# michaelriedl/2048-ppo-agent

Hardware: AMD Instinct MI355X
Metric: env-steps/sec at N parallel boards (full PPO loop: rollout with policy in the loop + GAE + update) (higher is better)
Workload: dtype u8 boards / bf16 policy; 1 GPU; 65536 parallel boards per GPU, Transformer policy bf16 (3.96 M params), full PPO iteration (BASELINE.json configs[2]; configs[3] when n_gpus=8); boards_per_gpu=65536, global_boards=65536, train_batch=2048, update_epochs=5, max_samples_per_epoch=300000, max_samples_per_epoch_is=global (each rank draws its 1/N share), as the reference's single subset, max_samples_per_epoch_per_rank=300000, rollout_mode=episodes (reference lock-step semantics), rng_mode=partitionable, parallelism=env-shard x1 + 1 grad all-reduce/minibatch

## Files before the change

### 2048-ppo-agent_amd/csrc/g2048_policy.hip

```cpp
#include <hip/hip_runtime.h>
#include <stdint.h>

#include "../../include/g2048.h"
#include "g2048_host.h"
#include "g2048_mfma.h"

namespace {

using g2048_mfma::bf16x4;
using g2048_mfma::bf16x8;
using g2048_mfma::f32x16;
using g2048_mfma::f32x4;
using g2048_mfma::mfma;
using g2048_mfma::rowof;
using g2048_mfma::sched_fence;
using g2048_mfma::static_for;
using namespace g2048_host;

typedef short s16x2 __attribute__((ext_vector_type(2)));

constexpr int D = 256, NH = 8, HD = 32, FF = 1024, SEQ = 17, NBOARD = 7, NTOK = 128, THREADS = 256;
constexpr int W_LAYER = 3 * D * D + D * D + FF * D + D * FF;
constexpr int P_LAYER = D + D + 3 * D + D + D + D + FF + D;
constexpr int WO_QKV = 0, WO_O = 3 * D * D, WO_1 = WO_O + D * D, WO_2 = WO_1 + FF * D;
constexpr int PO_LN1G = 0, PO_LN1B = D, PO_BQKV = 2 * D, PO_BO = 5 * D, PO_LN2G = 6 * D, PO_LN2B = 7 * D,
              PO_B1 = 8 * D, PO_B2 = 8 * D + FF;
constexpr int FFC = 64;
constexpr int TILE = 32 * D * 2;
constexpr float SM_SCALE_LOG2E = 0.17677669529663687f * 1.4426950408889634f;

template <int CPR> __device__ __forceinline__ int swz(int r);
template <> __device__ __forceinline__ int swz<32>(int r) { return r & 15; }
template <> __device__ __forceinline__ int swz<16>(int r) { return r & 15; }
template <> __device__ __forceinline__ int swz<8>(int r) { return (r >> 1) & 7; }
template <> __device__ __forceinline__ int swz<4>(int r) { return (r >> 2) & 3; }

struct LaneOff {
    int a256[8];
    int a64[4];
    int a32[2];
    unsigned s256[2], s64, s32;
};
__device__ __forceinline__ void lane_offsets(LaneOff &o, int r, int h, int w, int lane) {
    for (int k = 0; k < 8; ++k) o.a256[k] = r * 512 + (((2 * k + h) ^ swz<32>(r)) * 16);
    for (int k = 0; k < 4; ++k) o.a64[k] = r * 128 + (((2 * k + h) ^ swz<8>(r)) * 16);
    for (int k = 0; k < 2; ++k) o.a32[k] = r * 64 + (((2 * k + h) ^ swz<4>(r)) * 16);
    for (int par = 0; par < 2; ++par) {
        const int x = 2 * w + (lane >> 5), row15 = (8 * par + x) & 15;
        o.s256[par] = (unsigned)(x * D * 2 + (((lane & 31) ^ row15) * 16));
    }
    {
        const int x = 8 * w + (lane >> 3);
        o.s64 = (unsigned)(x * FF * 2 + (((lane & 7) ^ swz<8>(x)) * 16));
    }
    {
        const int x = 16 * w + (lane >> 2);
        o.s32 = (unsigned)(x * D * 2 + (((lane & 3) ^ swz<4>(x)) * 16));
    }
}

template <int CPR>
__device__ __forceinline__ bf16x8 load_w(const char *tile, const LaneOff &o, int mt, int ks) {
    if (CPR == 32) return *reinterpret_cast<const bf16x8 *>(tile + o.a256[ks & 7] + (ks >> 3) * 256 + mt * 32 * 512);
    if (CPR == 8) return *reinterpret_cast<const bf16x8 *>(tile + o.a64[ks] + mt * 32 * 128);
    return *reinterpret_cast<const bf16x8 *>(tile + o.a32[ks] + mt * 32 * 64);
}
__device__ __forceinline__ bf16x8 load_p(const char *row, int ks, int h) {
    return *reinterpret_cast<const bf16x8 *>(row + 2 * (16 * ks + 8 * h));
}

__device__ __forceinline__ void frag_from_acc(const f32x16 &x, bf16x8 out[2]) {
    for (int s = 0; s < 2; ++s)
        for (int j = 0; j < 8; ++j) out[s][j] = (__bf16)x[8 * s + j];
}
__device__ __forceinline__ void relu_frag_from_acc(const f32x16 &x, bf16x8 out[2]) {
    frag_from_acc(x, out);
    for (int s = 0; s < 2; ++s) {
        s16x2 *p = reinterpret_cast<s16x2 *>(&out[s]);
        const s16x2 zero = {0, 0};
        for (int q = 0; q < 4; ++q) p[q] = __builtin_elementwise_max(p[q], zero);
    }
}

__device__ __forceinline__ f32x16 bias_tile(const float *b32, int h) {
    f32x16 a;
    for (int g = 0; g < 4; ++g) {
        const f32x4 v = *reinterpret_cast<const f32x4 *>(b32 + 8 * g + 4 * h);
        for (int q = 0; q < 4; ++q) a[4 * g + q] = v[q];
    }
    return a;
}

template <int CPR, int NK, bool SWAP = false>
__device__ __forceinline__ f32x16 gemm_tile(const char *tile, const LaneOff &o, int mt, const bf16x8 *b, f32x16 acc) {
    bf16x8 a[NK];
    for (int ks = 0; ks < NK; ++ks) a[ks] = load_w<CPR>(tile, o, mt, ks);
    for (int ks = 0; ks < NK; ++ks) acc = SWAP ? mfma(b[ks], a[ks], acc) : mfma(a[ks], b[ks], acc);
    return acc;
}
template <int NM, int EXTRA = 0, int NV = 0, int VALU_PER = 0, int TRANS_PER = 0, int DEPTH = 8>
__device__ __forceinline__ void pipe_mfma() {
    __builtin_amdgcn_sched_group_barrier(0x100, DEPTH + EXTRA, 0);
#pragma unroll
    for (int i = 0; i < NM; ++i) {
        __builtin_amdgcn_sched_group_barrier(0x008, 1, 0);
        if (i < NM - DEPTH) __builtin_amdgcn_sched_group_barrier(0x100, 1, 0);
        if (i < NV && VALU_PER) __builtin_amdgcn_sched_group_barrier(0x002, VALU_PER, 0);
        if (i < NV && TRANS_PER) __builtin_amdgcn_sched_group_barrier(0x400, TRANS_PER, 0);
    }
}

#ifdef G2048_STAMPS
constexpr int N_STAMPS = 24;
__device__ unsigned long long g_stamps[N_STAMPS];
struct StampSite {
    __device__ __forceinline__ static bool on(int lane, int w) { return lane == 0 && w == 0 && blockIdx.x % 64 == 0; }
    __device__ __forceinline__ static unsigned long long *table(int) { return g_stamps; }
};
#define STAMP(k) stamps.mark(k)
#else
#define STAMP(k)
#endif

typedef __amdgpu_buffer_rsrc_t rsrc_t;
template <int CPR>
__device__ __forceinline__ void dma_tile(char *dst, rsrc_t blob, unsigned src_byte, int ld, int rows, const LaneOff &o, int w) {
    const int n_inst = rows * CPR / (64 * 4);
    const int rows_per_inst = 4 * 64 / CPR;
    for (int t = 0; t < n_inst; ++t) {
        const unsigned lane_off = CPR == 32 ? o.s256[t & 1] : (CPR == 8 ? o.s64 : o.s32);
        __builtin_amdgcn_raw_ptr_buffer_load_lds(blob, (__attribute__((address_space(3))) void *)(dst + (t * 4 + w) * 1024), 16,
                                                 (int)lane_off, (int)(src_byte + (unsigned)(t * rows_per_inst * ld * 2)), 0, 0);
    }
}
template <int CPR>
__device__ __forceinline__ void dma_inst(char *dst, rsrc_t blob, unsigned src_byte, int ld, int t, const LaneOff &o, int w) {
    const int rows_per_inst = 4 * 64 / CPR;
    const unsigned lane_off = CPR == 32 ? o.s256[t & 1] : (CPR == 8 ? o.s64 : o.s32);
    __builtin_amdgcn_raw_ptr_buffer_load_lds(blob, (__attribute__((address_space(3))) void *)(dst + (t * 4 + w) * 1024), 16,
                                             (int)lane_off, (int)(src_byte + (unsigned)(t * rows_per_inst * ld * 2)), 0, 0);
}
template <int N> __device__ __forceinline__ void dma_wait() { asm volatile("s_waitcnt vmcnt(%0)" ::"n"(N) : "memory"); }
__device__ __forceinline__ void dma_wait_all() { dma_wait<0>(); }

__device__ __forceinline__ void stage_f32(float *dst, const float *src, int n, int tid) {
    for (int i = tid; i < n; i += THREADS) dst[i] = src[i];
}

__device__ __forceinline__ void park_in_agpr(bf16x8 &x) { asm volatile("" : "+a"(x)); }

__device__ __forceinline__ float xhalf_sum(float x) {
    const auto r = __builtin_amdgcn_permlane32_swap(__float_as_uint(x), __float_as_uint(x), false, false);
    return __uint_as_float(r[0]) + __uint_as_float(r[1]);
}
__device__ __forceinline__ float xhalf_max(float x) {
    const auto r = __builtin_amdgcn_permlane32_swap(__float_as_uint(x), __float_as_uint(x), false, false);
    return fmaxf(__uint_as_float(r[0]), __uint_as_float(r[1]));
}

__device__ __forceinline__ void layer_norm(const f32x16 r[8], bf16x8 out[16]) {
    typedef float f32x2 __attribute__((ext_vector_type(2)));
    f32x2 s2[4], q2[4];
    for (int k = 0; k < 4; ++k) s2[k] = q2[k] = f32x2{0.f, 0.f};
    for (int j = 0; j < 8; ++j)
        for (int i = 0; i < 16; i += 2) {
            const f32x2 v = {r[j][i], r[j][i + 1]};
            const int k = (i >> 1) & 3;
            s2[k] += v;
            q2[k] = __builtin_elementwise_fma(v, v, q2[k]);
        }
    const f32x2 st = (s2[0] + s2[1]) + (s2[2] + s2[3]), qt = (q2[0] + q2[1]) + (q2[2] + q2[3]);
    float s = st[0] + st[1], ss = qt[0] + qt[1];
    s = xhalf_sum(s);
    ss = xhalf_sum(ss);
    const float mean = s * (1.0f / D);
    const float var = fmaxf(__builtin_fmaf(-mean, mean, ss * (1.0f / D)), 0.0f);
    const float rstd = rsqrtf(var + 1e-5f), shift = -mean * rstd;
    for (int j = 0; j < 8; ++j)
        for (int i = 0; i < 16; ++i) out[2 * j + (i >> 3)][i & 7] = (__bf16)__builtin_fmaf(r[j][i], rstd, shift);
    for (int k = 0; k < 16; ++k) park_in_agpr(out[k]);
}

constexpr int MODE_FULL = 0, MODE_HEAD = 1, MODE_MEAN = 2;
constexpr int64_t KV_ELEMS = (int64_t)NH * SEQ * HD;

constexpr int L_WQKV = 0;
constexpr int L_WO = 6 * TILE;
constexpr int L_K = 7 * TILE;
constexpr int L_VT = 7 * TILE + TILE / 2;
constexpr int L_W1 = 0;
constexpr int L_W2 = 4 * TILE;
struct LdsMain {
    char w[8 * TILE];
    float bq[D], bo[D], b1[FF], b2[D];
};
static_assert(sizeof(LdsMain) <= 160 * 1024, "LDS budget");
constexpr int MEAN_LD = D + 4;
static_assert(NBOARD * 16 * MEAN_LD * 4 <= (int)sizeof(LdsMain::w), "mean-pool stage fits over the weight area");

template <int MODE>
__global__ void __launch_bounds__(THREADS, 1)
k_encoder_main(const uint8_t *__restrict__ boards, const float *__restrict__ table, const float *__restrict__ cls,
               const __bf16 *__restrict__ wblob, const float *__restrict__ pblob, int n_layers,
               float *__restrict__ features, int64_t B, __bf16 *__restrict__ ws_k, __bf16 *__restrict__ ws_v,
               float *__restrict__ ws_r) {
    extern __shared__ __attribute__((aligned(16))) char smem[];
    LdsMain &L = *reinterpret_cast<LdsMain *>(smem);
    const int tid = threadIdx.x, lane = tid & 63, r = lane & 31, h = lane >> 5;
    const int w = __builtin_amdgcn_readfirstlane(tid >> 6);
    const int64_t board0 = (int64_t)blockIdx.x * NBOARD;
    LaneOff lo;
    lane_offsets(lo, r, h, w, lane);

    const int tok = 32 * w + r;
    const int tb = tok / SEQ;
    const int tc = tok - tb * SEQ;
    const bool tok_valid = tb < NBOARD && board0 + tb < B;

    const int kb = w == 0 ? 0 : (w == 1 ? 16 : (w == 2 ? 48 : 64));
    int k_rd[2], vt_rd[4], k_wr[2], vt_wr[2];
    for (int ks = 0; ks < 2; ++ks) k_rd[ks] = L_K + kb * 64 + lo.a32[ks];
    for (int ks = 0; ks < 4; ++ks) vt_rd[ks] = L_VT + r * 256 + (((kb / 8 + 2 * ks + h) ^ swz<16>(r)) * 16);
    for (int s = 0; s < 2; ++s) {
        k_wr[s] = L_K + tok * 64 + (((2 * s + h) ^ swz<4>(tok)) * 16);
        vt_wr[s] = L_VT + r * 256 + (((4 * w + 2 * s + h) ^ swz<16>(r)) * 16);
    }
    bf16x8 kmask[2], qmask;
    {
        const int qb = tb;
        for (int j = 0; j < 8; ++j) qmask[j] = (__bf16)((qb == 8 * h + j) ? 16.0f : 0.0f);
        for (int tl = 0; tl < 2; ++tl) {
            const int kbd = (kb + 32 * tl + r) / SEQ;
            for (int j = 0; j < 8; ++j) kmask[tl][j] = (__bf16)((kbd == 8 * h + j) ? 16.0f : 0.0f);
        }
        park_in_agpr(qmask);
        park_in_agpr(kmask[0]);
        park_in_agpr(kmask[1]);
    }

    f32x16 R[8];
    {
        const float *src = cls;
        if (tok_valid && tc != 0) {
            int e = boards[(board0 + tb) * 16 + (tc - 1)];
            e = e > 30 ? 30 : e;
            src = table + ((size_t)(tc - 1) * 31 + e) * D;
        }
        const float keep = tok_valid ? 1.0f : 0.0f;
        for (int j = 0; j < 8; ++j)
            for (int g = 0; g < 4; ++g) {
                const f32x4 v = *reinterpret_cast<const f32x4 *>(src + 32 * j + 8 * g + 4 * h);
                for (int q = 0; q < 4; ++q) R[j][4 * g + q] = keep * v[q];
            }
    }

    const int full_layers = MODE == MODE_HEAD ? n_layers - 1 : n_layers;
    char *const lds = L.w;
    const rsrc_t blob = __builtin_amdgcn_make_buffer_rsrc(const_cast<__bf16 *>(wblob), 0, n_layers * (W_LAYER * 2), 0x00020000);
    auto wqkv = [&](int hd) -> char * { return lds + L_WQKV + (hd & 1) * 3 * TILE; };
    auto dma_qkv1 = [&](unsigned lw, int hd, int n) __attribute__((always_inline)) {
        dma_inst<32>(wqkv(hd) + (n / 4) * TILE, blob, lw + 2u * (unsigned)(WO_QKV + ((n / 4) * D + HD * hd) * D), D, n % 4, lo, w);
    };
    auto dma_wo1 = [&](unsigned lw, int hd, int n) __attribute__((always_inline)) {
        dma_inst<4>(lds + L_WO, blob, lw + 2u * (unsigned)(WO_O + HD * hd), D, n, lo, w);
    };
    auto dma_w11 = [&](unsigned lw, int c, int n) __attribute__((always_inline)) {
        dma_inst<32>(lds + L_W1 + (c & 1) * 2 * TILE, blob, lw + 2u * (unsigned)(WO_1 + FFC * c * D), D, n, lo, w);
    };
    auto dma_w21 = [&](unsigned lw, int c, int n) __attribute__((always_inline)) {
        dma_inst<8>(lds + L_W2 + (c & 1) * 2 * TILE, blob, lw + 2u * (unsigned)(WO_2 + FFC * c), FF, n, lo, w);
    };

#ifdef G2048_STAMPS
    g2048_mfma::Stamps<N_STAMPS, StampSite> stamps;
    stamps.start();
#endif
    for (int n = 0; n < 12; ++n) dma_qkv1(0u, 0, n);
    for (int n = 0; n < 12; ++n) dma_qkv1(0u, 1, n);

    constexpr int PD = 8;
    bf16x8 xn[16];
#pragma nounroll
    for (int layer = 0; layer < full_layers; ++layer) {
        const unsigned lw = (unsigned)layer * (unsigned)(W_LAYER * 2);
        const float *P = pblob + (size_t)layer * P_LAYER;

        float stg[7];
        stg[0] = P[PO_BQKV + tid];
        stg[1] = P[PO_BO + tid];
        stg[2] = P[PO_B2 + tid];
        for (int q = 0; q < 4; ++q) stg[3 + q] = P[PO_B1 + 256 * q + tid];
        layer_norm(R, xn);
        L.bq[tid] = stg[0];
        L.bo[tid] = stg[1];
        L.b2[tid] = stg[2];
        for (int q = 0; q < 4; ++q) L.b1[256 * q + tid] = stg[3 + q];
        dma_wait_all();
        __syncthreads();
        STAMP(0);

        f32x16 qa, ka, va;
        bf16x8 qf[2], kf[2], vf[2];
        auto project = [&](int hd, auto softmax_tag, auto fetch, f32x16 &s0, f32x16 &s1, bf16x8 *pf, float &sum) __attribute__((always_inline)) {
            constexpr bool SOFTMAX = decltype(softmax_tag)::value;
            const char *t = wqkv(hd);
            bf16x8 a[PD];
            qa = bias_tile(L.bq + HD * hd, h);
            for (int i = 0; i < 16; ++i) ka[i] = va[i] = 0.f;
            static_for<0, PD>([&](auto ic) __attribute__((always_inline)) {
                constexpr int i = decltype(ic)::value;
                a[i] = load_w<32>(t + (i / 16) * TILE, lo, 0, i % 16);
            });
            float m = 0.f, mc = 0.f;
            sched_fence();
            static_for<0, 48>([&](auto ic) __attribute__((always_inline)) {
                constexpr int i = decltype(ic)::value;
                constexpr int ks = i % 16;
                if constexpr (i < 16) qa = mfma(a[i % PD], xn[ks], qa);
                else if constexpr (i < 32) ka = mfma(a[i % PD], xn[ks], ka);
                else va = mfma(xn[ks], a[i % PD], va);
                if constexpr (i + PD < 48) a[i % PD] = load_w<32>(t + ((i + PD) / 16) * TILE, lo, 0, (i + PD) % 16);
                if constexpr (i % 3 == 0) fetch(std::integral_constant<int, i / 3>{});
                if constexpr (SOFTMAX) {
                    if constexpr (i < 8) {
                        const float x = fmaxf(fmaxf(s0[2 * i], s0[2 * i + 1]), fmaxf(s1[2 * i], s1[2 * i + 1]));
                        m = i == 0 ? x : fmaxf(m, x);
                    } else if constexpr (i == 8) {
                        m = xhalf_max(m);
                        mc = -m * SM_SCALE_LOG2E;
                        sum = 0.f;
                    } else if constexpr (i < 41) {
                        constexpr int e = i - 9;
                        if constexpr (e < 16) {
                            s0[e] = __builtin_amdgcn_exp2f(__builtin_fmaf(s0[e], SM_SCALE_LOG2E, mc));
                            sum += s0[e];
                        } else {
                            s1[e - 16] = __builtin_amdgcn_exp2f(__builtin_fmaf(s1[e - 16], SM_SCALE_LOG2E, mc));
                            sum += s1[e - 16];
                        }
                    } else if constexpr (i == 41) {
                        sum = xhalf_sum(sum);
                    } else if constexpr (i < 46) {
                        constexpr int k = i - 42;
                        for (int j = 0; j < 8; ++j) {
                            if constexpr (k < 2) pf[k][j] = (__bf16)s0[8 * (k & 1) + j];
                            else pf[k][j] = (__bf16)s1[8 * (k & 1) + j];
                        }
                    }
                }
                sched_fence();
            });
        };
        auto pack_qkv = [&](auto nc) __attribute__((always_inline)) {
            constexpr int n = decltype(nc)::value, which = n / 4, s = (n / 2) & 1, half = n & 1;
            for (int j = 0; j < 4; ++j) {
                if constexpr (which == 0) qf[s][4 * half + j] = (__bf16)qa[8 * s + 4 * half + j];
                else if constexpr (which == 1) kf[s][4 * half + j] = (__bf16)ka[8 * s + 4 * half + j];
                else vf[s][4 * half + j] = (__bf16)va[8 * s + 4 * half + j];
            }
        };
        auto store_kv = [&]() __attribute__((always_inline)) {
            for (int s = 0; s < 2; ++s) {
                *reinterpret_cast<bf16x8 *>(lds + k_wr[s]) = kf[s];
                *reinterpret_cast<bf16x8 *>(lds + vt_wr[s]) = vf[s];
            }
        };
        {
            f32x16 d0, d1;
            float dsum;
            project(0, std::false_type{}, [](auto) {}, d0, d1, nullptr, dsum);
            static_for<0, 12>(pack_qkv);
        }
        store_kv();
        __syncthreads();
        STAMP(1);

        auto head = [&](int hd, auto next_tag) __attribute__((always_inline)) {
            constexpr int NEXT = decltype(next_tag)::value;
            bf16x8 kr[4];
            for (int ks = 0; ks < 2; ++ks) {
                kr[2 * ks] = *reinterpret_cast<const bf16x8 *>(lds + k_rd[ks]);
                kr[2 * ks + 1] = *reinterpret_cast<const bf16x8 *>(lds + k_rd[ks] + 32 * 64);
            }
            sched_fence();
            auto fetch = [&](auto nc) __attribute__((always_inline)) {
                constexpr int n = decltype(nc)::value;
                if constexpr (n < 4) dma_wo1(lw, hd, n);
                else if constexpr (NEXT == 0) dma_qkv1(lw, hd + 2, n - 4);
                else if constexpr (NEXT == 1 && n < 12) dma_w11(lw, 0, n - 4);
            };
            if constexpr (NEXT == 2) static_for<0, 4>(fetch);
            sched_fence();
            STAMP(2);
            f32x16 s0 = {0}, s1 = {0};
            for (int ks = 0; ks < 2; ++ks) {
                s0 = mfma(kr[2 * ks], qf[ks], s0);
                s1 = mfma(kr[2 * ks + 1], qf[ks], s1);
            }
            s0 = mfma(kmask[0], qmask, s0);
            s1 = mfma(kmask[1], qmask, s1);
            sched_fence();
            STAMP(3);
            bf16x8 pf[4];
            float sum;
            if constexpr (NEXT != 2) {
                project(hd + 1, std::true_type{}, fetch, s0, s1, pf, sum);
            } else {
                float m = fmaxf(s0[0], s1[0]);
                for (int i = 1; i < 16; ++i) m = fmaxf(m, fmaxf(s0[i], s1[i]));
                m = xhalf_max(m);
                const float mc = -m * SM_SCALE_LOG2E;
                sum = 0.f;
                for (int i = 0; i < 16; ++i) {
                    s0[i] = __builtin_amdgcn_exp2f(__builtin_fmaf(s0[i], SM_SCALE_LOG2E, mc));
                    s1[i] = __builtin_amdgcn_exp2f(__builtin_fmaf(s1[i], SM_SCALE_LOG2E, mc));
                    sum += s0[i] + s1[i];
                }
                sum = xhalf_sum(sum);
                frag_from_acc(s0, pf);
                frag_from_acc(s1, pf + 2);
            }
            sched_fence();
            STAMP(4);
            f32x16 o = {0};
            for (int ks = 0; ks < 4; ++ks) o = mfma(*reinterpret_cast<const bf16x8 *>(lds + vt_rd[ks]), pf[ks], o);
            const float inv = __builtin_amdgcn_rcpf(sum);
            for (int i = 0; i < 16; ++i) o[i] *= inv;
            bf16x8 of[2];
            frag_from_acc(o, of);
            STAMP(5);
            if constexpr (NEXT == 0) dma_wait<12>();
            if constexpr (NEXT == 1) dma_wait<8>();
            if constexpr (NEXT == 2) dma_wait<0>();
            asm volatile("s_waitcnt lgkmcnt(0)" ::: "memory");
            __builtin_amdgcn_s_barrier();
            sched_fence();
            STAMP(6);
            {
                const char *wo = lds + L_WO;
                bf16x8 a[PD];
                static_for<0, PD>([&](auto ic) __attribute__((always_inline)) {
                    constexpr int i = decltype(ic)::value;
                    a[i] = load_w<4>(wo, lo, i / 2, i % 2);
                });
                sched_fence();
                static_for<0, 16>([&](auto ic) __attribute__((always_inline)) {
                    constexpr int i = decltype(ic)::value;
                    R[i / 2] = mfma(a[i % PD], of[i % 2], R[i / 2]);
                    if constexpr (i + PD < 16) a[i % PD] = load_w<4>(wo, lo, (i + PD) / 2, (i + PD) % 2);
                    if constexpr (NEXT != 2 && i < 12) pack_qkv(ic);
                    if constexpr (NEXT != 2 && i == 12) store_kv();
                    sched_fence();
                });
            }
            STAMP(7);
            dma_wait_all();
            STAMP(8);
            __syncthreads();
            STAMP(9);
        };
#pragma nounroll
        for (int hd = 0; hd < NH - 2; ++hd) head(hd, std::integral_constant<int, 0>{});
        head(NH - 2, std::integral_constant<int, 1>{});
        head(NH - 1, std::integral_constant<int, 2>{});

        for (int j = 0; j < 8; ++j) {
            dma_w11(lw, 1, j);
            const f32x16 b = bias_tile(L.bo + 32 * j, h);
            for (int i = 0; i < 16; ++i) R[j][i] += b[i];
        }
        layer_norm(R, xn);
        STAMP(10);
        f32x16 hA0, hA1, hB0, hB1;
        bf16x8 hf[4];
        auto pack_h = [&](auto nc, const f32x16 &g0, const f32x16 &g1) __attribute__((always_inline)) {
            constexpr int n = decltype(nc)::value, k = n / 4, q = n % 4;
            for (int j = 0; j < 2; ++j) {
                if constexpr (k < 2) hf[k][2 * q + j] = (__bf16)g0[8 * (k & 1) + 2 * q + j];
                else hf[k][2 * q + j] = (__bf16)g1[8 * (k & 1) + 2 * q + j];
            }
            if constexpr (q == 3) {
                s16x2 *p2 = reinterpret_cast<s16x2 *>(&hf[k]);
                const s16x2 zero = {0, 0};
                for (int u = 0; u < 4; ++u) p2[u] = __builtin_elementwise_max(p2[u], zero);
            }
        };
        auto ffn_chain = [&](auto with1_tag, auto with2_tag, int c1, int c2, f32x16 &n0, f32x16 &n1, const f32x16 &g0, const f32x16 &g1,
                             auto fetch) __attribute__((always_inline)) {
            constexpr bool WITH1 = decltype(with1_tag)::value, WITH2 = decltype(with2_tag)::value;
            constexpr int N1 = WITH1 ? 32 : 0, NS = N1 + (WITH2 ? 32 : 0);
            const char *t1 = lds + L_W1 + (c1 & 1) * 2 * TILE, *t2 = lds + L_W2 + (c2 & 1) * 2 * TILE;
            if constexpr (WITH1) {
                n0 = bias_tile(L.b1 + FFC * c1, h);
                n1 = bias_tile(L.b1 + FFC * c1 + 32, h);
            }
            bf16x8 a[PD];
            auto rd = [&](auto sc) __attribute__((always_inline)) {
                constexpr int s = decltype(sc)::value;
                if constexpr (s < N1) a[s % PD] = load_w<32>(t1, lo, s / 16, s % 16);
                else a[s % PD] = load_w<8>(t2, lo, (s - N1) / 4, (s - N1) % 4);
            };
            static_for<0, PD>(rd);
            if constexpr (!WITH1 && WITH2) static_for<0, 16>([&](auto nc) __attribute__((always_inline)) { pack_h(nc, g0, g1); });
            sched_fence();
            static_for<0, NS>([&](auto ic) __attribute__((always_inline)) {
                constexpr int i = decltype(ic)::value;
                if constexpr (i < N1) {
                    if constexpr (i < 16) n0 = mfma(a[i % PD], xn[i % 16], n0);
                    else n1 = mfma(a[i % PD], xn[i % 16], n1);
                } else {
                    R[(i - N1) / 4] = mfma(a[i % PD], hf[(i - N1) % 4], R[(i - N1) / 4]);
                }
                if constexpr (i + PD < NS) rd(std::integral_constant<int, i + PD>{});
                if constexpr (NS == 64 ? (i % 3 == 0 && i < 48) : i % 2 == 0) fetch(std::integral_constant<int, NS == 64 ? i / 3 : i / 2>{});
                if constexpr (WITH1 && WITH2 && i < 16) pack_h(ic, g0, g1);
                sched_fence();
            });
        };
        {
            f32x16 dummy0, dummy1;
            ffn_chain(std::true_type{}, std::false_type{}, 0, 0, hA0, hA1, dummy0, dummy1, [&](auto nc) __attribute__((always_inline)) {
                constexpr int n = decltype(nc)::value;
                if constexpr (n < 8) dma_w21(lw, 0, n);
            });
        }
        dma_wait_all();
        __syncthreads();
        STAMP(11);
        auto chunk = [&](int c, auto last_tag, f32x16 &n0, f32x16 &n1, const f32x16 &g0, const f32x16 &g1) __attribute__((always_inline)) {
            constexpr int LAST = decltype(last_tag)::value;
            auto fetch = [&](auto nc) __attribute__((always_inline)) {
                constexpr int n = decltype(nc)::value;
                if constexpr (LAST == 0) {
                    if constexpr (n < 8) dma_w11(lw, c + 2, n);
                    else dma_w21(lw, c + 1, n - 8);
                } else if constexpr (LAST == 1) {
                    if constexpr (n < 8) dma_w21(lw, c + 1, n);
                    else dma_qkv1(lw + W_LAYER * 2, 0, n - 8);
                } else {
                    if constexpr (n < 4) dma_qkv1(lw + W_LAYER * 2, 0, 8 + n);
                    else dma_qkv1(lw + W_LAYER * 2, 1, n - 4);
                }
            };
            STAMP(12);
            if constexpr (LAST != 2) ffn_chain(std::true_type{}, std::true_type{}, c + 1, c, n0, n1, g0, g1, fetch);
            else ffn_chain(std::false_type{}, std::true_type{}, 0, c, n0, n1, g0, g1, fetch);
            STAMP(14);
            if constexpr (LAST == 2)
                for (int j = 0; j < 8; ++j) {
                    const f32x16 b = bias_tile(L.b2 + 32 * j, h);
                    for (int i = 0; i < 16; ++i) R[j][i] += b[i];
                }
            dma_wait_all();
            STAMP(15);
            __syncthreads();
            STAMP(16);
        };
#pragma nounroll
        for (int c = 0; c < FF / FFC - 2; c += 2) {
            chunk(c, std::integral_constant<int, 0>{}, hB0, hB1, hA0, hA1);
            chunk(c + 1, std::integral_constant<int, 0>{}, hA0, hA1, hB0, hB1);
        }
        chunk(FF / FFC - 2, std::integral_constant<int, 1>{}, hB0, hB1, hA0, hA1);
        chunk(FF / FFC - 1, std::integral_constant<int, 2>{}, hA0, hA1, hB0, hB1);
    }

    STAMP(17);
    if (MODE == MODE_HEAD) {
        const unsigned lwl = (unsigned)(n_layers - 1) * (unsigned)(W_LAYER * 2);
        if (tok_valid && tc == 0) {
            float *dst = ws_r + (board0 + tb) * D;
            for (int j = 0; j < 8; ++j)
                for (int g = 0; g < 4; ++g) {
                    f32x4 v;
                    for (int q = 0; q < 4; ++q) v[q] = R[j][4 * g + q];
                    *reinterpret_cast<f32x4 *>(dst + 32 * j + 8 * g + 4 * h) = v;
                }
        }
        layer_norm(R, xn);
        dma_wait_all();
        __syncthreads();
        bf16x8 kst[2], vst[2];
        auto store_head = [&](int hd) __attribute__((always_inline)) {
            if (tok_valid) {
                const size_t off = (size_t)(board0 + tb) * KV_ELEMS + ((size_t)hd * SEQ + tc) * HD + 16 * h;
                *reinterpret_cast<bf16x8 *>(ws_k + off) = kst[0];
                *reinterpret_cast<bf16x8 *>(ws_k + off + 8) = kst[1];
                *reinterpret_cast<bf16x8 *>(ws_v + off) = vst[0];
                *reinterpret_cast<bf16x8 *>(ws_v + off + 8) = vst[1];
            }
        };
        auto kv_head = [&](int hd, auto fetch_tag, auto store_tag) __attribute__((always_inline)) {
            constexpr bool FETCH = decltype(fetch_tag)::value, STORE = decltype(store_tag)::value;
            if constexpr (STORE) store_head(hd - 1);
            const char *t = wqkv(hd);
            f32x16 ka2 = {0}, va2 = {0};
            bf16x8 a[PD];
            static_for<0, PD>([&](auto ic) __attribute__((always_inline)) {
                constexpr int i = decltype(ic)::value;
                a[i] = load_w<32>(t + (1 + i / 16) * TILE, lo, 0, i % 16);
            });
            sched_fence();
            static_for<0, 32>([&](auto ic) __attribute__((always_inline)) {
                constexpr int i = decltype(ic)::value;
                if constexpr (i < 16) ka2 = mfma(a[i % PD], xn[i % 16], ka2);
                else va2 = mfma(a[i % PD], xn[i % 16], va2);
                if constexpr (i + PD < 32) a[i % PD] = load_w<32>(t + (1 + (i + PD) / 16) * TILE, lo, 0, (i + PD) % 16);
                if constexpr (FETCH && i % 3 == 0 && i < 24) dma_qkv1(lwl, hd + 1, 4 + i / 3);
                if constexpr (i >= 20 && i < 22)
                    for (int j = 0; j < 8; ++j) kst[i - 20][j] = (__bf16)ka2[8 * (i - 20) + j];
                sched_fence();
            });
            frag_from_acc(va2, vst);
            dma_wait_all();
            __syncthreads();
        };
        kv_head(0, std::false_type{}, std::false_type{});
#pragma nounroll
        for (int hd = 1; hd < NH - 1; ++hd) kv_head(hd, std::true_type{}, std::true_type{});
        kv_head(NH - 1, std::false_type{}, std::true_type{});
        store_head(NH - 1);
        STAMP(18);
#ifdef G2048_STAMPS
        stamps.flush(lane, w);
#endif
        return;
    }

    if constexpr (MODE == MODE_MEAN) {
        dma_wait_all();
        __syncthreads();
        const int ln = (int)__builtin_amdgcn_mbcnt_hi(~0u, __builtin_amdgcn_mbcnt_lo(~0u, 0u));
        const int t = 64 * w + ln, mtok = 32 * w + (ln & 31), mtb = mtok / SEQ, mtc = mtok - mtb * SEQ, mh = ln >> 5;
        float *const stage = reinterpret_cast<float *>(lds);
        if (mtb < NBOARD && board0 + mtb < B && mtc != 0) {
            float *dst = stage + (mtb * 16 + mtc - 1) * MEAN_LD;
            for (int j = 0; j < 8; ++j)
                for (int g = 0; g < 4; ++g) {
                    f32x4 v;
                    for (int q = 0; q < 4; ++q) v[q] = R[j][4 * g + q];
                    *reinterpret_cast<f32x4 *>(dst + 32 * j + 8 * g + 4 * mh) = v;
                }
        }
        __syncthreads();
        for (int b = 0; b < NBOARD && board0 + b < B; ++b) {
            const float *src = stage + b * 16 * MEAN_LD + t;
            float s = 0.f;
            for (int k = 0; k < 16; ++k) s += src[k * MEAN_LD];
            features[(board0 + b) * D + t] = s * 0.0625f;
        }
    } else {
        if (tok_valid && tc == 0) {
            float *dst = features + (board0 + tb) * D;
            for (int j = 0; j < 8; ++j)
                for (int g = 0; g < 4; ++g) {
                    f32x4 v;
                    for (int q = 0; q < 4; ++q) v[q] = R[j][4 * g + q];
                    *reinterpret_cast<f32x4 *>(dst + 32 * j + 8 * g + 4 * h) = v;
                }
        }
    }
}

constexpr int ST32 = 2 * 32 + 16;
struct LdsTail {
    char w[6 * TILE];
    char w2b[2 * TILE];
    char o[NTOK * ST32];
    float bias[FF];
};
static_assert(sizeof(LdsTail) <= 160 * 1024, "LDS budget");

__global__ void __launch_bounds__(THREADS, 1)
k_encoder_tail(const __bf16 *__restrict__ wblob, const float *__restrict__ pblob, int n_layers, float *__restrict__ features,
               int64_t B, const __bf16 *__restrict__ ws_k, const __bf16 *__restrict__ ws_v, const float *__restrict__ ws_r) {
    extern __shared__ __attribute__((aligned(16))) char smem[];
    LdsTail &L = *reinterpret_cast<LdsTail *>(smem);
    const int tid = threadIdx.x, lane = tid & 63, r = lane & 31, h = lane >> 5;
    const int w = __builtin_amdgcn_readfirstlane(tid >> 6);
    const int64_t board0 = (int64_t)blockIdx.x * NTOK;
    char *const wq = L.w;
    LaneOff lo;
    lane_offsets(lo, r, h, w, lane);
    const int tok = 32 * w + r;
    const bool tok_valid = board0 + tok < B;
    const int64_t my_board = tok_valid ? board0 + tok : (B - 1);

    f32x16 R[8];
    {
        const float *src = ws_r + my_board * D;
        for (int j = 0; j < 8; ++j)
            for (int g = 0; g < 4; ++g) {
                const f32x4 v = *reinterpret_cast<const f32x4 *>(src + 32 * j + 8 * g + 4 * h);
                for (int q = 0; q < 4; ++q) R[j][4 * g + q] = v[q];
            }
    }
    const rsrc_t blob = __builtin_amdgcn_make_buffer_rsrc(const_cast<__bf16 *>(wblob), 0, n_layers * (W_LAYER * 2), 0x00020000);
    const unsigned lw = (unsigned)(n_layers - 1) * (unsigned)(W_LAYER * 2);
    const float *P = pblob + (size_t)(n_layers - 1) * P_LAYER;
    auto dma_q = [&](int hd) { dma_tile<32>(wq, blob, lw + 2u * (unsigned)(WO_QKV + HD * hd * D), D, HD, lo, w); };
    auto wo_of = [&](int hd) -> char * { return L.w + (3 + (hd & 1)) * TILE; };
    auto dma_wo = [&](int hd) { dma_tile<4>(wo_of(hd), blob, lw + 2u * (unsigned)(WO_O + HD * hd), D, D, lo, w); };

    dma_q(0);
    dma_wo(0);
    stage_f32(L.bias, P + PO_BQKV, D, tid);
    bf16x8 xn[16];
    layer_norm(R, xn);
    dma_wait_all();
    __syncthreads();
#pragma nounroll
    for (int hd = 0; hd < NH; ++hd) {
        f32x16 qa = gemm_tile<32, 16>(wq, lo, 0, xn, bias_tile(L.bias + HD * hd, h));
        pipe_mfma<16>();
        const size_t off = (size_t)my_board * KV_ELEMS + (size_t)hd * SEQ * HD + 16 * h;
        float sc[SEQ], m = -3.0e38f;
        for (int key = 0; key < SEQ; ++key) {
            const bf16x8 k0 = *reinterpret_cast<const bf16x8 *>(ws_k + off + key * HD);
            const bf16x8 k1 = *reinterpret_cast<const bf16x8 *>(ws_k + off + key * HD + 8);
            float d = 0.f;
            for (int i = 0; i < 8; ++i) d += (float)(__bf16)qa[i] * (float)k0[i] + (float)(__bf16)qa[8 + i] * (float)k1[i];
            d = xhalf_sum(d);
            sc[key] = d * 0.17677669529663687f;
            m = fmaxf(m, sc[key]);
        }
        float sum = 0.f;
        for (int key = 0; key < SEQ; ++key) {
            sc[key] = __expf(sc[key] - m);
            sum += sc[key];
        }
        const float inv = 1.0f / sum;
        float o[16];
        for (int i = 0; i < 16; ++i) o[i] = 0.f;
        for (int key = 0; key < SEQ; ++key) {
            const bf16x8 v0 = *reinterpret_cast<const bf16x8 *>(ws_v + off + key * HD);
            const bf16x8 v1 = *reinterpret_cast<const bf16x8 *>(ws_v + off + key * HD + 8);
            const float p = (float)(__bf16)sc[key];
            for (int i = 0; i < 8; ++i) {
                o[i] += p * (float)v0[i];
                o[8 + i] += p * (float)v1[i];
            }
        }
        for (int s = 0; s < 2; ++s) {
            bf16x8 ov;
            for (int q = 0; q < 8; ++q) ov[q] = (__bf16)(o[8 * s + q] * inv);
            *reinterpret_cast<bf16x8 *>(L.o + tok * ST32 + 2 * (16 * s + 8 * h)) = ov;
        }
        __syncthreads();
        if (hd + 1 < NH) {
            dma_q(hd + 1);
            dma_wo(hd + 1);
        }
        bf16x8 of[2];
        for (int ks = 0; ks < 2; ++ks) of[ks] = load_p(L.o + tok * ST32, ks, h);
        const char *wo = wo_of(hd);
        for (int j = 0; j < 8; ++j) R[j] = gemm_tile<4, 2>(wo, lo, j, of, R[j]);
        pipe_mfma<16>();
        dma_wait_all();
        __syncthreads();
    }

    auto w1_of = [&](int c) -> char * { return L.w + ((c & 1) ? 2 * TILE : 0); };
    auto w2_of = [&](int c) -> char * { return (c & 1) ? L.w2b : L.w + 4 * TILE; };
    auto dma_ffn = [&](int c) {
        dma_tile<32>(w1_of(c), blob, lw + 2u * (unsigned)(WO_1 + FFC * c * D), D, FFC, lo, w);
        dma_tile<8>(w2_of(c), blob, lw + 2u * (unsigned)(WO_2 + FFC * c), FF, D, lo, w);
    };
    dma_ffn(0);
    stage_f32(L.bias, P + PO_BO, D, tid);
    __syncthreads();
    for (int j = 0; j < 8; ++j) {
        const f32x16 b = bias_tile(L.bias + 32 * j, h);
        for (int i = 0; i < 16; ++i) R[j][i] += b[i];
    }
    layer_norm(R, xn);
    __syncthreads();
    stage_f32(L.bias, P + PO_B1, FF, tid);
    dma_wait_all();
    __syncthreads();
#pragma nounroll
    for (int c = 0; c < FF / FFC; ++c) {
        if (c + 1 < FF / FFC) dma_ffn(c + 1);
        const char *t1 = w1_of(c), *t2 = w2_of(c);
        f32x16 h0 = gemm_tile<32, 16>(t1, lo, 0, xn, bias_tile(L.bias + FFC * c, h));
        f32x16 h1 = gemm_tile<32, 16>(t1, lo, 1, xn, bias_tile(L.bias + FFC * c + 32, h));
        pipe_mfma<32>();
        bf16x8 hf[4];
        relu_frag_from_acc(h0, hf);
        relu_frag_from_acc(h1, hf + 2);
        for (int j = 0; j < 8; ++j) R[j] = gemm_tile<8, 4>(t2, lo, j, hf, R[j]);
        pipe_mfma<32>();
        dma_wait_all();
        __syncthreads();
    }
    if (tok_valid) {
        float *dst = features + (board0 + tok) * D;
        for (int j = 0; j < 8; ++j)
            for (int g = 0; g < 4; ++g) {
                const f32x4 b = *reinterpret_cast<const f32x4 *>(P + PO_B2 + 32 * j + 8 * g + 4 * h);
                f32x4 v;
                for (int q = 0; q < 4; ++q) v[q] = R[j][4 * g + q] + b[q];
                *reinterpret_cast<f32x4 *>(dst + 32 * j + 8 * g + 4 * h) = v;
            }
    }
}

}

#ifdef G2048_STAMPS
extern "C" int g2048_debug_stamps(unsigned long long *out , int reset) {
    if (hipMemcpyFromSymbol(out, HIP_SYMBOL(g_stamps), sizeof(unsigned long long) * N_STAMPS) != hipSuccess) return -1;
    if (reset) {
        unsigned long long z[N_STAMPS] = {0};
        if (hipMemcpyToSymbol(HIP_SYMBOL(g_stamps), z, sizeof(z)) != hipSuccess) return -1;
    }
    return N_STAMPS;
}
#endif

extern "C" int64_t g2048_policy_encoder_workspace_bytes(int64_t B) {
    return B <= 0 ? 0 : B * (2 * KV_ELEMS * (int64_t)sizeof(__bf16) + D * (int64_t)sizeof(float));
}

extern "C" int g2048_policy_encoder(const uint8_t *boards, const float *embed_table, const float *cls_token,
                                    const void *weights_bf16, const float *params_f32, int n_layers,
                                    float *features, int64_t B, void *workspace, void *stream) {
    if (!boards || !embed_table || !cls_token || !weights_bf16 || !params_f32 || !features || n_layers < 1 || B <= 0)
        return G2048_EINVAL;
    if (!aligned16(weights_bf16, params_f32, embed_table, cls_token, features, workspace)) return G2048_EINVAL;
    const void *main_fn = workspace ? reinterpret_cast<const void *>(k_encoder_main<MODE_HEAD>)
                                    : reinterpret_cast<const void *>(k_encoder_main<MODE_FULL>);
    if (const int rc = allow_dynamic_lds(main_fn, (int)sizeof(LdsMain))) return rc;
    if (workspace)
        if (const int rc = allow_dynamic_lds(reinterpret_cast<const void *>(k_encoder_tail), (int)sizeof(LdsTail))) return rc;
    const __bf16 *wb = reinterpret_cast<const __bf16 *>(weights_bf16);
    const unsigned blocks = (unsigned)((B + NBOARD - 1) / NBOARD);
    if (!workspace) {
        hipLaunchKernelGGL(k_encoder_main<MODE_FULL>, dim3(blocks), dim3(THREADS), sizeof(LdsMain), (hipStream_t)stream, boards,
                           embed_table, cls_token, wb, params_f32, n_layers, features, B, (__bf16 *)nullptr, (__bf16 *)nullptr,
                           (float *)nullptr);
    } else {
        __bf16 *ws_k = reinterpret_cast<__bf16 *>(workspace), *ws_v = ws_k + B * KV_ELEMS;
        float *ws_r = reinterpret_cast<float *>(ws_v + B * KV_ELEMS);
        hipLaunchKernelGGL(k_encoder_main<MODE_HEAD>, dim3(blocks), dim3(THREADS), sizeof(LdsMain), (hipStream_t)stream, boards,
                           embed_table, cls_token, wb, params_f32, n_layers, features, B, ws_k, ws_v, ws_r);
        hipLaunchKernelGGL(k_encoder_tail, dim3((unsigned)((B + NTOK - 1) / NTOK)), dim3(THREADS), sizeof(LdsTail),
                           (hipStream_t)stream, wb, params_f32, n_layers, features, B, ws_k, ws_v, ws_r);
    }
    return launch_status();
}

extern "C" int g2048_policy_encoder_mean(const uint8_t *boards, const float *embed_table, const float *cls_token,
                                         const void *weights_bf16, const float *params_f32, int n_layers, float *features,
                                         int64_t B, void *stream) {
    if (!boards || !embed_table || !cls_token || !weights_bf16 || !params_f32 || !features || n_layers < 1 || B <= 0)
        return G2048_EINVAL;
    if (!aligned16(weights_bf16, params_f32, embed_table, cls_token, features)) return G2048_EINVAL;
    if (const int rc = allow_dynamic_lds(reinterpret_cast<const void *>(k_encoder_main<MODE_MEAN>), (int)sizeof(LdsMain))) return rc;
    const unsigned blocks = (unsigned)((B + NBOARD - 1) / NBOARD);
    hipLaunchKernelGGL(k_encoder_main<MODE_MEAN>, dim3(blocks), dim3(THREADS), sizeof(LdsMain), (hipStream_t)stream, boards,
                       embed_table, cls_token, reinterpret_cast<const __bf16 *>(weights_bf16), params_f32, n_layers, features, B,
                       (__bf16 *)nullptr, (__bf16 *)nullptr, (float *)nullptr);
    return launch_status();
}
```

Baseline: 3.897 million env-steps/sec.

## Compute last-layer CLS attention in main kernel, write only CLS output to workspace

Adds a MODE_CLS path where the main encoder kernel handles the last layer's attention for just the CLS query. It computes Q for CLS, plus K/V and a per-head softmax inline, and writes a 256-wide bf16 attention output per board instead of full K/V for all 17 tokens. The tail kernel then only applies the out-projection and the FFN. This is meant to remove the large K/V workspace write and read plus the tail's per-head attention work, at the cost of extra LDS staging and scalar softmax work in the main kernel. The old path stays available behind an env var.

```diff
diff --git a/2048-ppo-agent_amd/csrc/g2048_policy.hip b/2048-ppo-agent_amd/csrc/g2048_policy.hip
--- a/2048-ppo-agent_amd/csrc/g2048_policy.hip
+++ b/2048-ppo-agent_amd/csrc/g2048_policy.hip
@@ -1,5 +1,7 @@
 #include <hip/hip_runtime.h>
+#include <stddef.h>
 #include <stdint.h>
+#include <stdlib.h>
 
 #include "../../include/g2048.h"
 #include "g2048_host.h"
@@ -181,7 +183,7 @@
     for (int k = 0; k < 16; ++k) park_in_agpr(out[k]);
 }
 
-constexpr int MODE_FULL = 0, MODE_HEAD = 1, MODE_MEAN = 2;
+constexpr int MODE_FULL = 0, MODE_HEAD = 1, MODE_MEAN = 2, MODE_CLS = 3;
 constexpr int64_t KV_ELEMS = (int64_t)NH * SEQ * HD;
 
 constexpr int L_WQKV = 0;
@@ -190,6 +192,12 @@
 constexpr int L_VT = 7 * TILE + TILE / 2;
 constexpr int L_W1 = 0;
 constexpr int L_W2 = 4 * TILE;
+constexpr int L_CX = 6 * TILE;
+constexpr int L_CQ = L_CX + 4096;
+constexpr int L_CS = L_CQ + 1024;
+constexpr int L_CO = L_CS + 1280;
+constexpr int L_CV = 7 * TILE;
+static_assert(L_CO + (NBOARD + 1) * D * 2 <= L_CV && L_CV + 2 * NTOK * HD * 2 <= 8 * TILE, "CLS staging fits the free tiles");
 struct LdsMain {
     char w[8 * TILE];
     float bq[D], bo[D], b1[FF], b2[D];
@@ -254,7 +262,7 @@
             }
     }
 
-    const int full_layers = MODE == MODE_HEAD ? n_layers - 1 : n_layers;
+    const int full_layers = (MODE == MODE_HEAD || MODE == MODE_CLS) ? n_layers - 1 : n_layers;
     char *const lds = L.w;
     const rsrc_t blob = __builtin_amdgcn_make_buffer_rsrc(const_cast<__bf16 *>(wblob), 0, n_layers * (W_LAYER * 2), 0x00020000);
     auto wqkv = [&](int hd) -> char * { return lds + L_WQKV + (hd & 1) * 3 * TILE; };
@@ -627,6 +635,147 @@
         return;
     }
 
+    if constexpr (MODE == MODE_CLS) {
+        const unsigned lwl = (unsigned)(n_layers - 1) * (unsigned)(W_LAYER * 2);
+        const float bq_stage = pblob[(size_t)(n_layers - 1) * P_LAYER + PO_BQKV + tid];
+        __bf16 *const ws_o = ws_k;
+        if (tok_valid && tc == 0) {
+            float *dst = ws_r + (board0 + tb) * D;
+            for (int j = 0; j < 8; ++j)
+                for (int g = 0; g < 4; ++g) {
+                    f32x4 v;
+                    for (int q = 0; q < 4; ++q) v[q] = R[j][4 * g + q];
+                    *reinterpret_cast<f32x4 *>(dst + 32 * j + 8 * g + 4 * h) = v;
+                }
+        }
+        layer_norm(R, xn);
+        L.bq[tid] = bq_stage;
+        if (tb < NBOARD && tc == 0)
+            for (int ks = 0; ks < 16; ++ks) *reinterpret_cast<bf16x8 *>(lds + L_CX + ((2 * ks + h) * 8 + tb) * 16) = xn[ks];
+        dma_wait_all();
+        __syncthreads();
+        const int sb = 2 * w + h;
+        const int sbc = sb < NBOARD ? sb : 0;
+        bf16x8 kst[2], vst[2];
+        constexpr std::true_type yes{};
+        constexpr std::false_type no{};
+        auto cls_head = [&](int it, auto kv_tag, auto fetch_tag, auto score_tag, auto soft_tag) __attribute__((always_inline)) {
+            constexpr bool KV = decltype(kv_tag)::value, FETCH = decltype(fetch_tag)::value;
+            constexpr bool SCORE = decltype(score_tag)::value, SOFT = decltype(soft_tag)::value;
+            const int pb = (it - 1) & 1, sbuf = it & 1;
+            bf16x8 q0, q1;
+            float d = 0.f, scv[SEQ], m = -3.0e38f, sum = 0.f, o = 0.f;
+            __bf16 vv[SEQ];
+            if constexpr (SCORE) {
+                q0 = *reinterpret_cast<const bf16x8 *>(lds + L_CQ + pb * 512 + tb * 64 + h * 32);
+                q1 = *reinterpret_cast<const bf16x8 *>(lds + L_CQ + pb * 512 + tb * 64 + h * 32 + 16);
+            }
+            if constexpr (SOFT) {
+                const char *src = lds + L_CS + (sbuf * 160 + sbc * 20) * 4;
+                for (int g = 0; g < 4; ++g) {
+                    const f32x4 v = *reinterpret_cast<const f32x4 *>(src + 16 * g);
+                    for (int q = 0; q < 4; ++q) scv[4 * g + q] = v[q];
+                }
+                scv[16] = *reinterpret_cast<const float *>(src + 64);
+            }
+            auto piece = [&](auto ic) __attribute__((always_inline)) {
+                constexpr int i = decltype(ic)::value;
+                if constexpr (SCORE) {
+                    if constexpr (i == 0) {
+                        for (int s = 0; s < 2; ++s)
+                            *reinterpret_cast<bf16x8 *>(lds + L_CV + pb * (NTOK * HD * 2) + tok * (HD * 2) + (16 * s + 8 * h) * 2) = vst[s];
+                    }
+                    if constexpr (i < 8) {
+                        d += (float)q0[i] * (float)kst[0][i] + (float)q1[i] * (float)kst[1][i];
+                    } else if constexpr (i == 8) {
+                        d = xhalf_sum(d);
+                        *reinterpret_cast<float *>(lds + L_CS + (pb * 160 + tb * 20 + tc) * 4) = d * 0.17677669529663687f;
+                    }
+                }
+                if constexpr (SOFT) {
+                    if constexpr (i < SEQ)
+                        vv[i] = *reinterpret_cast<const __bf16 *>(lds + L_CV + sbuf * (NTOK * HD * 2) + (SEQ * sbc + i) * (HD * 2) + r * 2);
+                    if constexpr (i == 9) {
+                        for (int key = 0; key < SEQ; ++key) m = fmaxf(m, scv[key]);
+                    } else if constexpr (i >= 10 && i < 10 + SEQ) {
+                        constexpr int key = i - 10;
+                        scv[key] = __expf(scv[key] - m);
+                        sum += scv[key];
+                        const float p = (float)(__bf16)scv[key];
+                        o += p * (float)vv[key];
+                    } else if constexpr (i == 10 + SEQ) {
+                        const float inv = 1.0f / sum;
+                        *reinterpret_cast<__bf16 *>(lds + L_CO + sb * (D * 2) + ((it - 2) * HD + r) * 2) = (__bf16)(o * inv);
+                    }
+                }
+            };
+            if constexpr (KV) {
+                auto chain = [&](auto qw_tag) __attribute__((always_inline)) {
+                    constexpr bool QW = decltype(qw_tag)::value;
+                    constexpr int NQ = QW ? 16 : 0, NS = NQ + 32;
+                    const char *t = wqkv(it);
+                    const char *xsrc = lds + L_CX + (h * 8 + (r & 7)) * 16;
+                    f32x16 ka2 = {0}, va2 = {0}, qa = {0};
+                    if constexpr (QW) qa = bias_tile(L.bq + HD * it, h);
+                    bf16x8 a[PD], bx[PD];
+                    auto rd = [&](auto sc) __attribute__((always_inline)) {
+                        constexpr int s = decltype(sc)::value;
+                        if constexpr (s < NQ) {
+                            a[s % PD] = load_w<32>(t, lo, 0, s);
+                            bx[s % PD] = *reinterpret_cast<const bf16x8 *>(xsrc + s * 256);
+                        } else {
+                            a[s % PD] = load_w<32>(t + (1 + (s - NQ) / 16) * TILE, lo, 0, (s - NQ) % 16);
+                        }
+                    };
+                    static_for<0, PD>(rd);
+                    sched_fence();
+                    static_for<0, NS>([&](auto ic) __attribute__((always_inline)) {
+                        constexpr int i = decltype(ic)::value, j = i - NQ;
+                        if constexpr (i < NQ) qa = mfma(a[i % PD], bx[i % PD], qa);
+                        else if constexpr (j < 16) ka2 = mfma(a[i % PD], xn[j], ka2);
+                        else va2 = mfma(a[i % PD], xn[j - 16], va2);
+                        if constexpr (i + PD < NS) rd(std::integral_constant<int, i + PD>{});
+                        if constexpr (FETCH && i % 2 == 0 && i < 24) dma_qkv1(lwl, it + 1, i / 2);
+                        if constexpr (i < 32) piece(ic);
+                        if constexpr (j >= 20 && j < 22)
+                            for (int e = 0; e < 8; ++e) kst[j - 20][e] = (__bf16)ka2[8 * (j - 20) + e];
+                        sched_fence();
+                    });
+                    frag_from_acc(va2, vst);
+                    if constexpr (QW) {
+                        if (r < NBOARD)
+                            for (int s = 0; s < 2; ++s) {
+                                bf16x8 qv;
+                                for (int e = 0; e < 8; ++e) qv[e] = (__bf16)qa[8 * s + e];
+                                *reinterpret_cast<bf16x8 *>(lds + L_CQ + (it & 1) * 512 + r * 64 + h * 32 + 16 * s) = qv;
+                            }
+                    }
+                };
+                if (w == (it & 3)) chain(yes);
+                else chain(no);
+            } else {
+                static_for<0, 32>(piece);
+            }
+            dma_wait_all();
+            __syncthreads();
+        };
+        cls_head(0, yes, no, no, no);
+        cls_head(1, yes, yes, yes, no);
+#pragma nounroll
+        for (int it = 2; it < NH - 1; ++it) cls_head(it, yes, yes, yes, yes);
+        cls_head(NH - 1, yes, no, yes, yes);
+        cls_head(NH, no, no, yes, yes);
+        cls_head(NH + 1, no, no, no, yes);
+        if (tid < NBOARD * 32 && board0 + (tid >> 5) < B)
+            *reinterpret_cast<bf16x8 *>(ws_o + (board0 + (tid >> 5)) * D + (tid & 31) * 8) =
+                *reinterpret_cast<const bf16x8 *>(lds + L_CO + (tid >> 5) * (D * 2) + (tid & 31) * 16);
+        STAMP(18);
+#ifdef G2048_STAMPS
+        stamps.flush(lane, w);
+#endif
+        return;
+    }
+
     if constexpr (MODE == MODE_MEAN) {
         dma_wait_all();
         __syncthreads();
@@ -670,7 +819,9 @@
     float bias[FF];
 };
 static_assert(sizeof(LdsTail) <= 160 * 1024, "LDS budget");
-
+static_assert(offsetof(LdsTail, w2b) == 6 * TILE, "w and w2b are one 8-tile area (the whole out_proj.weight)");
+
+template <bool KVWS>
 __global__ void __launch_bounds__(THREADS, 1)
 k_encoder_tail(const __bf16 *__restrict__ wblob, const float *__restrict__ pblob, int n_layers, float *__restrict__ features,
                int64_t B, const __bf16 *__restrict__ ws_k, const __bf16 *__restrict__ ws_v, const float *__restrict__ ws_r) {
@@ -702,10 +853,24 @@
     auto wo_of = [&](int hd) -> char * { return L.w + (3 + (hd & 1)) * TILE; };
     auto dma_wo = [&](int hd) { dma_tile<4>(wo_of(hd), blob, lw + 2u * (unsigned)(WO_O + HD * hd), D, D, lo, w); };
 
+    bf16x8 xn[16];
+    if constexpr (!KVWS) {
+        for (int hd = 0; hd < NH; ++hd) dma_tile<4>(L.w + hd * TILE, blob, lw + 2u * (unsigned)(WO_O + HD * hd), D, D, lo, w);
+        bf16x8 of[NH][2];
+        for (int hd = 0; hd < NH; ++hd)
+            for (int ks = 0; ks < 2; ++ks) of[hd][ks] = *reinterpret_cast<const bf16x8 *>(ws_k + my_board * D + hd * HD + 16 * ks + 8 * h);
+        dma_wait_all();
+        __syncthreads();
+#pragma unroll
+        for (int hd = 0; hd < NH; ++hd)
+            for (int j = 0; j < 8; ++j) R[j] = gemm_tile<4, 2>(L.w + hd * TILE, lo, j, of[hd], R[j]);
+        pipe_mfma<16 * NH>();
+        __syncthreads();
+    }
+    if constexpr (KVWS) {
     dma_q(0);
     dma_wo(0);
     stage_f32(L.bias, P + PO_BQKV, D, tid);
-    bf16x8 xn[16];
     layer_norm(R, xn);
     dma_wait_all();
     __syncthreads();
@@ -758,6 +923,7 @@
         pipe_mfma<16>();
         dma_wait_all();
         __syncthreads();
+    }
     }
 
     auto w1_of = [&](int c) -> char * { return L.w + ((c & 1) ? 2 * TILE : 0); };
@@ -828,23 +994,35 @@
     if (!boards || !embed_table || !cls_token || !weights_bf16 || !params_f32 || !features || n_layers < 1 || B <= 0)
         return G2048_EINVAL;
     if (!aligned16(weights_bf16, params_f32, embed_table, cls_token, features, workspace)) return G2048_EINVAL;
-    const void *main_fn = workspace ? reinterpret_cast<const void *>(k_encoder_main<MODE_HEAD>)
-                                    : reinterpret_cast<const void *>(k_encoder_main<MODE_FULL>);
+    const char *e = getenv("G2048_ENCODER_KV_WS");
+    const bool kv_ws = e && e[0] == '1';
+    const void *main_fn = !workspace ? reinterpret_cast<const void *>(k_encoder_main<MODE_FULL>)
+                          : kv_ws    ? reinterpret_cast<const void *>(k_encoder_main<MODE_HEAD>)
+                                     : reinterpret_cast<const void *>(k_encoder_main<MODE_CLS>);
+    const void *tail_fn = kv_ws ? reinterpret_cast<const void *>(k_encoder_tail<true>) : reinterpret_cast<const void *>(k_encoder_tail<false>);
     if (const int rc = allow_dynamic_lds(main_fn, (int)sizeof(LdsMain))) return rc;
     if (workspace)
-        if (const int rc = allow_dynamic_lds(reinterpret_cast<const void *>(k_encoder_tail), (int)sizeof(LdsTail))) return rc;
+        if (const int rc = allow_dynamic_lds(tail_fn, (int)sizeof(LdsTail))) return rc;
     const __bf16 *wb = reinterpret_cast<const __bf16 *>(weights_bf16);
     const unsigned blocks = (unsigned)((B + NBOARD - 1) / NBOARD);
     if (!workspace) {
         hipLaunchKernelGGL(k_encoder_main<MODE_FULL>, dim3(blocks), dim3(THREADS), sizeof(LdsMain), (hipStream_t)stream, boards,
                            embed_table, cls_token, wb, params_f32, n_layers, features, B, (__bf16 *)nullptr, (__bf16 *)nullptr,
                            (float *)nullptr);
+    } else if (!kv_ws) {
+        __bf16 *ws_o = reinterpret_cast<__bf16 *>(workspace);
+        float *ws_r = reinterpret_cast<float *>(ws_o + B * D);
+        hipLaunchKernelGGL(k_encoder_main<MODE_CLS>, dim3(blocks), dim3(THREADS), sizeof(LdsMain), (hipStream_t)stream, boards,
+                           embed_table, cls_token, wb, params_f32, n_layers, features, B, ws_o, (__bf16 *)nullptr, ws_r);
+        hipLaunchKernelGGL(k_encoder_tail<false>, dim3((unsigned)((B + NTOK - 1) / NTOK)), dim3(THREADS), sizeof(LdsTail),
+                           (hipStream_t)stream, wb, params_f32, n_layers, features, B, (const __bf16 *)ws_o, (const __bf16 *)nullptr,
+                           (const float *)ws_r);
     } else {
         __bf16 *ws_k = reinterpret_cast<__bf16 *>(workspace), *ws_v = ws_k + B * KV_ELEMS;
         float *ws_r = reinterpret_cast<float *>(ws_v + B * KV_ELEMS);
         hipLaunchKernelGGL(k_encoder_main<MODE_HEAD>, dim3(blocks), dim3(THREADS), sizeof(LdsMain), (hipStream_t)stream, boards,
                            embed_table, cls_token, wb, params_f32, n_layers, features, B, ws_k, ws_v, ws_r);
-        hipLaunchKernelGGL(k_encoder_tail, dim3((unsigned)((B + NTOK - 1) / NTOK)), dim3(THREADS), sizeof(LdsTail),
+        hipLaunchKernelGGL(k_encoder_tail<true>, dim3((unsigned)((B + NTOK - 1) / NTOK)), dim3(THREADS), sizeof(LdsTail),
                            (hipStream_t)stream, wb, params_f32, n_layers, features, B, ws_k, ws_v, ws_r);
     }
     return launch_status();
```

Measured after the change: 3.990 million env-steps/sec (median of 6 runs). 1.02x the previous value.
